# GestaltCogTeam/STEP

Measured on AMD Instinct MI355X. Metric: training windows/sec on PEMS04, horizon-12 MAE parity, 1/2/4/8 MI355X, higher is better.
Workload: dtype f16 (TSFormer Q/K/weights) + bf16 (P, V, GraphWaveNet / graph-learner GEMMs) operands, f32 accumulate

## Files before the change

include/step_hip.h:

```cpp
#ifndef STEP_HIP_H
#define STEP_HIP_H

#include <stdint.h>

#ifdef __cplusplus
extern "C" {
#endif

const char* step_last_error(void);
int step_abi_version(void);

typedef struct StepGemm {
    int M, N, K, batch;
    const void* A; long sam, sak, sab; int a_bf16;
    const void* B; long sbk, sbn, sbb; int b_bf16;
    float* C; long ldc, scn, scb;
    float alpha;
    int accumulate;
    const float* bias; int relu;
    int splitk;
    int a_kblk; long a_kstride;
    int b_kblk; long b_kstride;
    int b_nblk; long b_nstride;
    int c_nblk; long c_nstride;
// ... 37 lines not shown
    float *bn3_w, *bn3_b, *bn3_rm, *bn3_rv;
    float *fc_out_w, *fc_out_b;
    float *fc_cat_w, *fc_cat_b;
    int gemm_bf16;
} StepDglParams;

long step_dgl_global_saved_floats(int N, int T);
long step_dgl_global_work_floats(int N, int T, int backward);
int step_dgl_global_forward(const float* series_nt, int N, int T, const StepDglParams* p, int training,
                            float momentum, float* saved, float* work, float* g, void* stream);
int step_dgl_global_backward(const float* series_nt, int N, int T, const StepDglParams* p, const float* saved,
                             const float* dg, float* work, const StepDglParams* grads, void* stream);
#define STEP_DGL_FRESH_FC_GRAD 16
int step_dgl_global_backward_phase(const float* series_nt, int N, int T, const StepDglParams* p, const float* saved,
                             const float* dg, float* work, const StepDglParams* grads, int phase, void* stream);

typedef struct StepDglShard { int own1; double count1, count2; } StepDglShard;
int step_dgl_global_forward_shard(const float* series_slice, int N, int Ts, const StepDglParams* p, int training, float momentum,
                                  float* saved, float* work, double* sums, float* g, const StepDglShard* shard, int phase,
                                  void* stream);
int step_dgl_global_backward_shard(const float* series_slice, int N, int Ts, const StepDglParams* p, const float* saved,
                                   const float* dg, float* work, const StepDglParams* grads, const StepDglShard* shard, int phase,
                                   void* stream);
long step_dgl_global_offset(int N, int T, int item);

long step_dgl_edges_saved_floats(int B, int N);
long step_dgl_edges_work_floats(int N);
long step_dgl_edges_theta_offset(int N);
int step_dgl_edges_forward(const float* g, int N, int B, const StepDglParams* p, const float* u, uint64_t seed,
                           float temperature, float* saved, float* theta_out, float* adj_out, void* stream);
// ... 91 lines not shown
                               uint32_t* keepbits, const uint64_t* pool, long pool_words, void* stream);
int step_pt_attention_bwd_bf16(const uint16_t* qkv, const uint16_t* out, const uint16_t* dout, const float* stats, long S, int T, float p,
                               uint64_t seed, uint32_t site, uint16_t* dqkv, const uint32_t* keepbits, void* stream);
int step_pt_linear_bf16out(const float* x, const float* w, long swk, long swn, const float* bias, long R, int N, int K, uint16_t* out,
                           void* stream);
int step_pt_relu_mask(float* d, const float* y, long n, void* stream);
int step_colsum(const float* x, long rows, int cols, long ld, float* out, void* stream);

long step_adam_work_floats(void);
int step_adam_clip(float* params, const float* grads, float* exp_avg, float* exp_avg_sq, long n, float lr, float beta1,
                   float beta2, float eps, float weight_decay, int step, float max_norm, float* work, float* out_norm,
                   void* stream);
int step_adam_clip_sharded(float* params, const float* grads, float* exp_avg, float* exp_avg_sq, long n, float lr, float beta1,
                           float beta2, float eps, float weight_decay, int step, float max_norm, const float* extra_sumsq,
                           float* work, float* out_norm, void* stream);
int step_loss_fwd_bwd(const float* pred, const float* real, long n_pred, const float* theta, const float* prior, long n_adj,
                      float null_val, float coef, double* work, float* loss, float* dpred, float* dtheta, void* stream);
int step_loss_scaled_fwd_bwd(const float* pred, const float* real, long n_pred, long real_stride, float scale, float shift,
                             const float* theta, const float* prior, long n_adj, float null_val, float coef, double* work, float* loss,
                             float* dpred, float* dtheta, void* stream);
int step_masked_metrics(const float* pred, long pred_stride, const float* real, long real_stride, long n, float null_val, double* work,
                        float* out, void* stream);
int step_scale2(const float* a, long na, const float* b, long nb, const float* g, float* out_a, float* out_b, void* stream);

typedef struct StepDynState {
    uint64_t seed_xor;
    int32_t adam_step;
    float lr;
    float gsl_coef;
    float reserved;
// ... 67 lines not shown
```

step_amd/_lib.py:

```python
import ctypes
import os

import torch

_HERE = os.path.dirname(os.path.abspath(__file__))
LIB_PATH = os.environ.get("STEP_HIP_LIB") or os.path.join(_HERE, "libstep_hip.so")

_vp, _i, _l, _f, _u64 = ctypes.c_void_p, ctypes.c_int, ctypes.c_long, ctypes.c_float, ctypes.c_uint64


class StepGemm(ctypes.Structure):
    _fields_ = [("M", _i), ("N", _i), ("K", _i), ("batch", _i),
                ("A", _vp), ("sam", _l), ("sak", _l), ("sab", _l), ("a_bf16", _i),
                ("B", _vp), ("sbk", _l), ("sbn", _l), ("sbb", _l), ("b_bf16", _i),
                ("C", _vp), ("ldc", _l), ("scn", _l), ("scb", _l),
                ("alpha", _f), ("accumulate", _i), ("bias", _vp), ("relu", _i), ("splitk", _i),
                ("a_kblk", _i), ("a_kstride", _l), ("b_kblk", _i), ("b_kstride", _l),
                ("b_nblk", _i), ("b_nstride", _l), ("c_nblk", _i), ("c_nstride", _l),
                ("a_kscale", _vp), ("a_kshift", _vp), ("a_kperiod", _i),
                ("batch0", _i), ("sab1", _l), ("sbb1", _l), ("scb1", _l), ("compute_bf16", _i), ("a_rowsum", _vp), ("c_nscale", _vp), ("c_nshift", _vp), ("c_mvec", _vp),
                ("c_nperiod", _i), ("splitk_ws", _vp), ("splitk_ws_floats", _l)]


class StepDglParams(ctypes.Structure):
# ... 34 lines not shown
    "step_tsformer_encode": (_i, [_vp, _i, _i, _vp, _l, _i, _i, _vp, _vp, _vp, _vp, _f, _vp, _l, _u64, _vp, _vp]),
    "step_dropout_pool_fill": (_i, [_vp, _l, _f, _u64, _vp]),
    "step_tsformer_dropout_words": (_l, [_i, _i]),
    "step_gather_windows": (_i, [_vp, _i, _i, _i, _i, _vp, _i, _i, _i, _vp, _vp, _vp, _vp]),
    "step_pack_long_history": (_i, [_vp, _i, _i, _i, _i, _i, _vp, _vp]),
    "step_knn_workspace_bytes": (_l, [_i, _i, _i]),
    "step_knn_graph": (_i, [_vp, _vp, _i, _i, _i, _i, _vp, _vp, _vp, _l, _vp]),
    "step_topk_mask": (_i, [_vp, _i, _i, _i, _vp, _vp, _l, _vp]),
    "step_selftest_mfma": (_i, [_vp, _vp]),
    "step_streams_concurrent": (_i, [_vp, _vp, ctypes.POINTER(_i)]),
    "step_dgl_global_saved_floats": (_l, [_i, _i]),
    "step_dgl_global_work_floats": (_l, [_i, _i, _i]),
    "step_dgl_global_forward": (_i, [_vp, _i, _i, _PD, _i, _f, _vp, _vp, _vp, _vp]),
    "step_dgl_global_backward": (_i, [_vp, _i, _i, _PD, _vp, _vp, _vp, _PD, _vp]),
    "step_dgl_global_backward_phase": (_i, [_vp, _i, _i, _PD, _vp, _vp, _vp, _PD, _i, _vp]),
    "step_dgl_global_forward_shard": (_i, [_vp, _i, _i, _PD, _i, _f, _vp, _vp, _vp, _vp, _PS, _i, _vp]),
    "step_dgl_global_backward_shard": (_i, [_vp, _i, _i, _PD, _vp, _vp, _vp, _PD, _PS, _i, _vp]),
    "step_dgl_global_offset": (_l, [_i, _i, _i]),
    "step_dgl_edges_saved_floats": (_l, [_i, _i]),
    "step_dgl_edges_work_floats": (_l, [_i]),
    "step_dgl_edges_theta_offset": (_l, [_i]),
    "step_dgl_edges_forward": (_i, [_vp, _i, _i, _PD, _vp, _u64, _f, _vp, _vp, _vp, _vp]),
    "step_dgl_edges_forward_keyed": (_i, [_vp, _i, _i, _PD, _vp, _u64, _f, _vp, _vp, _vp, _vp]),
    "step_dgl_edges_backward": (_i, [_vp, _i, _i, _PD, _vp, _vp, _vp, _f, _vp, _PD, _vp, _vp, _vp]),
    "step_dgl_edges_backward_acc": (_i, [_vp, _i, _i, _PD, _vp, _vp, _vp, _f, _vp, _PD, _vp, _i, _vp, _vp]),
    "step_gwnet_saved_floats": (_l, [_i, _i, _i]),
    "step_gwnet_work_floats": (_l, [_i, _i, _i]),
    "step_gwnet_saved_offset": (_l, [_i, _i, _i, _i, _i]),
    "step_gwnet_forward": (_i, [_vp, _i, _i, _i, _vp, _vp, _PG, _i, _f, _u64, _f, _vp, _vp, _vp, _vp]),
    "step_gwnet_forward_phase": (_i, [_vp, _i, _i, _i, _vp, _vp, _PG, _i, _f, _u64, _f, _vp, _vp, _vp, _i, _vp]),
# ... 34 lines not shown
    "step_pt_layernorm_bwd": (_i, [_vp, _vp, _l, _vp, _vp, _vp, _vp, _vp, _vp]),
    "step_pt_attention_fwd": (_i, [_vp, _l, _i, _f, _u64, ctypes.c_uint32, _vp, _vp, _vp]),
    "step_pt_attention_bwd": (_i, [_vp, _vp, _vp, _vp, _l, _i, _f, _u64, ctypes.c_uint32, _vp, _vp]),
    "step_pt_attention_fwd_bf16": (_i, [_vp, _l, _i, _f, _u64, ctypes.c_uint32, _vp, _vp, _vp, _vp, _l, _vp]),
    "step_pt_attention_bwd_bf16": (_i, [_vp, _vp, _vp, _vp, _l, _i, _f, _u64, ctypes.c_uint32, _vp, _vp, _vp]),
    "step_pt_linear_bf16out": (_i, [_vp, _vp, _l, _l, _vp, _l, _i, _i, _vp, _vp]),
    "step_pt_relu_mask": (_i, [_vp, _vp, _l, _vp]),
    "step_colsum": (_i, [_vp, _l, _i, _l, _vp, _vp]),
    "step_loss_fwd_bwd": (_i, [_vp, _vp, _l, _vp, _vp, _l, _f, _f, _vp, _vp, _vp, _vp, _vp]),
    "step_loss_scaled_fwd_bwd": (_i, [_vp, _vp, _l, _l, _f, _f, _vp, _vp, _l, _f, _f, _vp, _vp, _vp, _vp, _vp]),
    "step_scale2": (_i, [_vp, _l, _vp, _l, _vp, _vp, _vp, _vp]),
    "step_masked_metrics": (_i, [_vp, _l, _vp, _l, _l, _f, _vp, _vp, _vp]),
    "step_adam_work_floats": (_l, []),
    "step_adam_clip": (_i, [_vp, _vp, _vp, _vp, _l, _f, _f, _f, _f, _f, _i, _f, _vp, _vp, _vp]),
    "step_adam_clip_sharded": (_i, [_vp, _vp, _vp, _vp, _l, _f, _f, _f, _f, _f, _i, _f, _vp, _vp, _vp, _vp]),
    "step_comm_available": (_i, []),
    "step_comm_version": (_i, []),
    "step_comm_unique_id": (_i, [_vp]),
    "step_comm_init_rank": (_i, [_vp, _i, _i, ctypes.POINTER(_vp)]),
    "step_comm_destroy": (_i, [_vp]),
    "step_comm_set_side_stream": (_i, [_vp, _vp]),
    "step_comm_allreduce": (_i, [_vp, _vp, _l, _i, _i, _vp]),
    "step_comm_broadcast": (_i, [_vp, _vp, _l, _i, _i, _vp]),
    "step_grad_allreduce": (_i, [_vp, _vp, _l, _vp]),
    "step_grad_allreduce_begin": (_i, [_vp, _vp, _l, _vp]),
    "step_grad_allreduce_join": (_i, [_vp, _vp]),
    "step_dyn_advance": (_i, [_vp, _vp]),
    "step_dropout_pool_fill_dyn": (_i, [_vp, _l, _f, _u64, _vp, _vp]),
    "step_dgl_edges_forward_dyn": (_i, [_vp, _i, _i, _PD, _vp, _u64, _f, _vp, _vp, _vp, _vp, _vp]),
    "step_gwnet_forward_phase_dyn": (_i, [_vp, _i, _i, _i, _vp, _vp, _PG, _i, _f, _u64, _f, _vp, _vp, _vp, _i, _vp, _vp]),
# ... 99 lines not shown
```

step_amd/csrc/dgl.hip:

```cpp
#include "common.h"
#include "step_internal.h"

namespace {

constexpr int KW = 10;
constexpr int EMB = 100;

template <int CI, int CO, int TPT>
__global__ __launch_bounds__(256) void conv_relu_fwd_kernel(const float* __restrict__ in, const float* __restrict__ w,
                                                            const float* __restrict__ b, const float* __restrict__ in_sc,
                                                            const float* __restrict__ in_sh, float* __restrict__ out,
                                                            float* __restrict__ partial, int Tin, int stat_limit) {
    __shared__ __attribute__((aligned(16))) float ws[CI * KW * CO];
    __shared__ float red[4][2 * CO];
    const int tid = threadIdx.x, n = blockIdx.y;
    const int Tout = Tin - (KW - 1);
    for (int e = tid; e < CI * KW * CO; e += 256) {
        int co = e % CO, k = (e / CO) % KW, ci = e / (CO * KW);
        ws[e] = w[(co * CI + ci) * KW + k];
    }
    __syncthreads();
    const int t0 = (blockIdx.x * 256 + tid) * TPT;
    float acc[CO][TPT];
#pragma unroll
// ... 156 lines not shown
            rvar[j] = (1.f - momentum) * rvar[j] + momentum * (float)(var * N / fmax((double)N - 1.0, 1.0));
        }
    } else {
        mean = rmean[j]; var = rvar[j];
    }
    const float rstd = (float)(1.0 / sqrt(var + 1e-5));
    if (tid == 0) { stat[2 * EMB + j] = (float)mean; stat[3 * EMB + j] = rstd; }
    const float sc = gamma[j] * rstd, sh = beta[j] - (float)mean * sc;
    for (int n = tid; n < N; n += 256) g[(long)n * EMB + j] = fmaxf(gpre[(long)n * EMB + j], 0.f) * sc + sh;
}

__global__ __launch_bounds__(256) void bn3_relu_bwd_kernel(const float* __restrict__ dg, const float* __restrict__ gpre, int N,
                                                           const float* __restrict__ gamma, const float* __restrict__ stat,
                                                           float* __restrict__ dgamma, float* __restrict__ dbeta,
                                                           float* __restrict__ dbias, float* __restrict__ dgpre,
                                                           float* __restrict__ dgpreT, float* __restrict__ colsum) {
    __shared__ double r1[256], r2[256];
    const int j = blockIdx.x, tid = threadIdx.x;
    const float mean = stat[2 * EMB + j], rstd = stat[3 * EMB + j];
    double a = 0.0, q = 0.0;
    for (int n = tid; n < N; n += 256) {
        float d = dg[(long)n * EMB + j];
        float xh = (fmaxf(gpre[(long)n * EMB + j], 0.f) - mean) * rstd;
        a += d; q += (double)d * xh;
    }
    r1[tid] = a; r2[tid] = q;
    __syncthreads();
    for (int s = 128; s > 0; s >>= 1) {
        if (tid < s) { r1[tid] += r1[tid + s]; r2[tid] += r2[tid + s]; }
        __syncthreads();
    }
    const float m1 = (float)(r1[0] / N), m2 = (float)(r2[0] / N);
    const float k = gamma[j] * rstd;
// ... 422 lines not shown
        uint4* dst = wp + ((long)o * T2 + t) * 2;
        dst[0] = make_uint4(pack_bf16x2(v[0], v[1]), pack_bf16x2(v[2], v[3]), pack_bf16x2(v[4], v[5]), pack_bf16x2(v[6], v[7]));
        dst[1] = make_uint4(pack_bf16x2(v[8], v[9]), pack_bf16x2(v[10], v[11]), pack_bf16x2(v[12], v[13]), pack_bf16x2(v[14], v[15]));
    }
    acc = wave_sum(acc);
    if ((tid & 63) == 0) red[tid >> 6] = acc;
    __syncthreads();
    if (tid == 0) atomicAdd(&shiftdot[o], red[0] + red[1] + red[2] + red[3]);
}
__global__ void gpre_init_kernel(float* __restrict__ gpre, const float* __restrict__ shiftdot, long n) {
    const long i = (long)blockIdx.x * 256 + threadIdx.x;
    if (i < n) gpre[i] = shiftdot[i % EMB];
}
__global__ __launch_bounds__(256) void fc_unpermute_kernel(const float* __restrict__ graw, const float* __restrict__ fc_w,
                                                           const float* __restrict__ st2, const float* __restrict__ colsum,
                                                           float* __restrict__ dfc_w, float* __restrict__ dots_o, int T2, int overwrite) {
    __shared__ float red[16][32];
    const int o = blockIdx.y, t = blockIdx.x * 256 + threadIdx.x, tid = threadIdx.x, lane = tid & 63, wave = tid >> 6;
    const float cso = colsum[o];
    float d[32];
#pragma unroll
    for (int i = 0; i < 32; ++i) d[i] = 0.f;
    if (t < T2) {
        const float4* src = (const float4*)(graw + ((long)o * T2 + t) * 16);
        const float4 g0 = src[0], g1 = src[1], g2 = src[2], g3 = src[3];
        const float g[16] = {g0.x, g0.y, g0.z, g0.w, g1.x, g1.y, g1.z, g1.w, g2.x, g2.y, g2.z, g2.w, g3.x, g3.y, g3.z, g3.w};
        float w[16], old[16];
#pragma unroll
        for (int c = 0; c < 16; ++c) { const long idx = ((long)o * 16 + c) * T2 + t; w[c] = fc_w[idx]; old[c] = overwrite ? 0.f : dfc_w[idx]; }
#pragma unroll
        for (int c = 0; c < 16; ++c) {
            dfc_w[((long)o * 16 + c) * T2 + t] = old[c] + st2[c] * g[c] + st2[16 + c] * cso;
            d[2 * c] = w[c] * g[c]; d[2 * c + 1] = w[c] * cso;
        }
    }
#pragma unroll
    for (int i = 0; i < 32; ++i) {
        const float v = row_sum_fast(d[i]);
        if ((lane & 15) == 15) red[4 * wave + (lane >> 4)][i] = v;
    }
    __syncthreads();
    if (tid < 32) {
        float v = 0.f;
#pragma unroll
        for (int r = 0; r < 16; ++r) v += red[r][tid];
        atomicAdd(&dots_o[o * 32 + tid], v);
    }
}
__global__ void dots_reduce_kernel(const float* __restrict__ dots_o, float* __restrict__ dots) {
    const int i = threadIdx.x;
    if (i >= 32) return;
    double a = 0.0;
    for (int o = 0; o < EMB; ++o) a += dots_o[o * 32 + i];
    dots[i] = (float)a;
}

static bool dgl_channels_last(const StepDglParams* p) {
    const char* e = getenv("STEP_DGL_F32_STORAGE");
    return p->gemm_bf16 && !(e && e[0] == '1');
}

static bool dgl_legacy_bn_backward() {
// ... 143 lines not shown
}

extern "C" long step_dgl_global_offset(int N, int T, int item) {
    const long T1 = T - 9, T2 = T - 18;
    if (item == 0) return 0;
    if (item == 1) return (long)N * 8 * T1;
    if (item == 2) return (long)N * 8 * T1 + (long)N * 16 * T2;
    const long nb1 = (long)N * cdiv(T1, 1024), nb2 = (long)N * cdiv(T2, 1024);
    const long coef = (nb1 > nb2 ? nb1 : nb2) * 32 + 64 + (long)N * 16 * T2 + (long)N * 8 * T1 + wraw_floats(T2) + 2L * N * EMB;
    if (item == 10) return coef + 256;
    if (item == 11) return coef + 320;
    return -1;
}

static int dgl_global_backward_impl(const float* series_nt, int N, int T, const StepDglParams* p, const float* saved, const float* dg,
                                    float* work, const StepDglParams* grads, const StepDglShard* shard, int phase, void* stream);

extern "C" int step_dgl_global_backward(const float* series_nt, int N, int T, const StepDglParams* p, const float* saved,
                                        const float* dg, float* work, const StepDglParams* grads, void* stream) {
    return step_dgl_global_backward_phase(series_nt, N, T, p, saved, dg, work, grads, 0, stream);
}

extern "C" int step_dgl_global_backward_phase(const float* series_nt, int N, int T, const StepDglParams* p, const float* saved,
                                              const float* dg, float* work, const StepDglParams* grads, int phase, void* stream) {
    STEP_REQUIRE(series_nt && p && saved && dg && work && grads && N > 0 && T > 18 && (phase & ~STEP_DGL_FRESH_FC_GRAD) >= 0 &&
                 (phase & ~STEP_DGL_FRESH_FC_GRAD) <= 2, "dgl_global_backward: bad arguments");
    return dgl_global_backward_impl(series_nt, N, T, p, saved, dg, work, grads, nullptr, phase, stream);
}

extern "C" int step_dgl_global_backward_shard(const float* series_slice, int N, int Ts, const StepDglParams* p, const float* saved,
                                              const float* dg, float* work, const StepDglParams* grads, const StepDglShard* shard,
                                              int phase, void* stream) {
    const int ph = phase & ~STEP_DGL_FRESH_FC_GRAD;
    STEP_REQUIRE(series_slice && p && saved && dg && work && grads && shard && N > 0 && Ts > 18 && (ph == 1 || ph == 3 || ph == 4),
                 "dgl_global_backward_shard: bad arguments");
    STEP_REQUIRE(p->gemm_bf16 && Ts - 18 >= 128, "dgl_global_backward_shard: needs the bf16 contraction mode and a slice of >= 128 conv2 columns");
    return dgl_global_backward_impl(series_slice, N, Ts, p, saved, dg, work, grads, shard, phase, stream);
}

static int dgl_global_backward_impl(const float* series_nt, int N, int T, const StepDglParams* p, const float* saved, const float* dg,
                                    float* work, const StepDglParams* grads, const StepDglShard* shard, int phase, void* stream) {
    const int fresh_fc = (phase & STEP_DGL_FRESH_FC_GRAD) ? 1 : 0;
    phase &= ~STEP_DGL_FRESH_FC_GRAD;
    const bool do_fc = phase == 0 || phase == 1, do_mid = phase == 0 || phase == 2 || phase == 3, do_tail = phase == 0 || phase == 2 || phase == 4;
    hipStream_t st = (hipStream_t)stream;
    const int T1 = T - 9, T2 = T - 18;
    const long K = 16L * T2;
    float *a1, *a2, *gpre, *st1, *st2, *st3;
    carve_saved((float*)saved, N, T, &a1, &a2, &gpre, &st1, &st2, &st3);
    long nb1 = (long)N * cdiv(T1, 1024), nb2 = (long)N * cdiv(T2, 1024);
    float* partial = work;
    float* d_a2 = work + (nb1 > nb2 ? nb1 : nb2) * 32 + 64;
    float* d_a1 = d_a2 + (long)N * 16 * T2;
    float* wraw = d_a1 + (long)N * 8 * T1;
    float* dgpre = wraw + wraw_floats(T2);
    float* dgpreT = dgpre + (long)N * EMB;
    float* coef = dgpreT + (long)N * EMB;
    float* dots = coef + 256;
    float* graw = coef + 320;
    float* wg_scratch = coef + DGL_SMALL;
    const bool fuse2 = T2 >= 128 && (shard || !dgl_legacy_bn_backward());
    const double count1 = shard ? shard->count1 : (double)N * T1, count2 = shard ? shard->count2 : (double)N * T2;
    if (dgl_channels_last(p)) {
        const float* wp = saved_wp((float*)saved, N, T);
        float* dots_o = coef + 256 + 64 + 1344;
        float* colsum = coef + 128;
        if (do_fc) {
            bn3_relu_bwd_kernel<<<EMB, 256, 0, st>>>(dg, gpre, N, p->bn3_w, st3, grads->bn3_w, grads->bn3_b, grads->fc_b, dgpre, dgpreT, colsum);
            STEP_LAUNCH_CHECK("bn3_bwd");
            StepGemm gm = gemm_desc(EMB, (int)K, N, dgpre, 1, EMB, a2, K, 1, wraw, K);
            gm.b_bf16 = 1;
            gm.compute_bf16 = 1;
            STEP_TRY(step_gemm_launch(gm, st));
            if (hipMemsetAsync(dots_o, 0, EMB * 32 * sizeof(float), st) != hipSuccess) { step_set_error("memset failed"); return STEP_ERR_HIP; }
            fc_unpermute_kernel<<<dim3(cdiv(T2, 256), EMB), 256, 0, st>>>(wraw, p->fc_w, st2, colsum, grads->fc_w, dots_o, T2, fresh_fc);
            dots_reduce_kernel<<<1, 64, 0, st>>>(dots_o, dots);
            STEP_LAUNCH_CHECK("fc_unpermute");
        }
        if (do_mid) {
            bn2_fused_coef_kernel<<<1, 64, 0, st>>>(dots, st2, p->bn2_w, count2, grads->bn2_w, grads->bn2_b, coef);
            STEP_LAUNCH_CHECK("bn2_fused_coef");
            StepGemm gm = gemm_desc(N, (int)K, EMB, dgpre, EMB, 1, wp, K, 1, d_a2, K);
            gm.b_bf16 = 1;
            gm.compute_bf16 = 1;
            GemmFused fu = {nullptr, nullptr, a2, coef, st2, 16, T2, GEMM_FUSED_INTERLEAVED};
            STEP_TRY(step_gemm_launch_fused(gm, fu, st));
            STEP_TRY(dgl_conv2_wgrad_cl(d_a2, a1, wg_scratch, graw, N, T1, st));
        }
        if (do_tail) {
            STEP_TRY(dgl_conv2_wgrad_finish(graw, p->conv2_w, st1, p->bn1_w, p->bn1_b, count1, grads->conv2_w, grads->conv2_b, grads->bn1_w,
                                            grads->bn1_b, coef + 64, 1, st));
            STEP_TRY(dgl_conv2_dgrad_cl(d_a2, p->conv2_w, st1, d_a1, N, T1, a1, coef + 64, st1, shard ? shard->own1 : T1, wraw, st));
            STEP_TRY(dgl_conv1_wgrad_cl(d_a1, series_nt, wg_scratch, grads->conv1_w, grads->conv1_b, N, T, st));
        }
        return STEP_OK;
    }
    if (do_fc) {
        float* colsum = coef + 128;
        bn3_relu_bwd_kernel<<<EMB, 256, 0, st>>>(dg, gpre, N, p->bn3_w, st3, grads->bn3_w, grads->bn3_b, grads->fc_b, dgpre, dgpreT, colsum);
        STEP_LAUNCH_CHECK("bn3_bwd");
        {
            StepGemm gm = gemm_desc(EMB, (int)K, N, dgpre, 1, EMB, a2, K, 1, grads->fc_w, K);
            gm.accumulate = fresh_fc ? 0 : 1;
            gm.c_nscale = st2; gm.c_nshift = st2 + 16; gm.c_nperiod = T2; gm.c_mvec = colsum;
            gm.compute_bf16 = p->gemm_bf16;
            if (fuse2) {
                if (hipMemsetAsync(dots, 0, 32 * sizeof(float), st) != hipSuccess) { step_set_error("memset failed"); return STEP_ERR_HIP; }
                GemmFused fu = {p->fc_w, dots, nullptr, nullptr, nullptr, 16, T2};
                STEP_TRY(step_gemm_launch_fused(gm, fu, st));
            } else {
                STEP_TRY(step_gemm_launch(gm, st));
            }
        }
    }
// ... 175 lines not shown
```

step_amd/csrc/optim.hip:

```cpp
#include "common.h"
#include "step_internal.h"
#include "tail_device.h"

namespace {

constexpr int NB = 1024;

__global__ __launch_bounds__(256) void sumsq_partial_kernel(const float* __restrict__ g, long n, float* __restrict__ partial) {
    __shared__ float red[4];
    float s = 0.f;
    const long n4 = n / 4;
    const float4* g4 = (const float4*)g;
    for (long i = (long)blockIdx.x * 256 + threadIdx.x; i < n4; i += (long)gridDim.x * 256) {
        float4 v = g4[i];
        s += v.x * v.x + v.y * v.y + v.z * v.z + v.w * v.w;
    }
    if (blockIdx.x == 0)
        for (long i = n4 * 4 + threadIdx.x; i < n; i += 256) s += g[i] * g[i];
    s = wave_sum(s);
    if ((threadIdx.x & 63) == 0) red[threadIdx.x >> 6] = s;
    __syncthreads();
    if (threadIdx.x == 0) partial[blockIdx.x] = red[0] + red[1] + red[2] + red[3];
}

__global__ __launch_bounds__(256) void adam_clip_kernel(float* __restrict__ p, const float* __restrict__ g, float* __restrict__ m,
                                                        float* __restrict__ v, long n, float lr, float beta1, float beta2, float eps,
                                                        float wd, float bc1, float bc2_sqrt, float max_norm,
                                                        const float* __restrict__ partial, int npartial, const float* __restrict__ extra_sumsq,
                                                        float* __restrict__ out_norm, const StepDynState* __restrict__ dyn) {
    __shared__ float red[4];
    __shared__ float s_coef;
    if (dyn) {
        const float t = (float)dyn->adam_step;
        lr = dyn->lr;
        bc1 = 1.f - powf(beta1, t);
        bc2_sqrt = sqrtf(1.f - powf(beta2, t));
    }
    {
        float s = 0.f;
        for (int i = threadIdx.x; i < npartial; i += 256) s += partial[i];
        s = wave_sum(s);
        if ((threadIdx.x & 63) == 0) red[threadIdx.x >> 6] = s;
        __syncthreads();
        if (threadIdx.x == 0) {
            const bool given = max_norm < 0.f;
            const float mx = given ? -max_norm : max_norm;
            const float norm = sqrtf(given ? *extra_sumsq : red[0] + red[1] + red[2] + red[3] + (extra_sumsq ? *extra_sumsq : 0.f));
            float c = mx > 0.f ? mx / (norm + 1e-6f) : 1.f;
            s_coef = c < 1.f ? c : 1.f;
            if (out_norm && blockIdx.x == 0) *out_norm = norm;
        }
        __syncthreads();
    }
    const float coef = s_coef;
    const float step_size = lr / bc1;
    for (long i = (long)blockIdx.x * 256 + threadIdx.x; i < n; i += (long)gridDim.x * 256) {
        const float pi = p[i];
        const float gi = g[i] * coef + wd * pi;
        const float mi = beta1 * m[i] + (1.f - beta1) * gi;
        const float vi = beta2 * v[i] + (1.f - beta2) * gi * gi;
        m[i] = mi; v[i] = vi;
        p[i] = pi - step_size * mi / (sqrtf(vi) / bc2_sqrt + eps);
// ... 1 lines not shown
}

}

extern "C" long step_adam_work_floats(void) { return NB + 8; }

extern "C" int step_adam_clip(float* params, const float* grads, float* exp_avg, float* exp_avg_sq, long n, float lr, float beta1,
                              float beta2, float eps, float weight_decay, int step, float max_norm, float* work, float* out_norm,
                              void* stream) {
    return step_adam_clip_sharded(params, grads, exp_avg, exp_avg_sq, n, lr, beta1, beta2, eps, weight_decay, step, max_norm, nullptr, work,
                                  out_norm, stream);
}

static int adam_clip_launch(float* params, const float* grads, float* exp_avg, float* exp_avg_sq, long n, float lr, float beta1,
                            float beta2, float eps, float weight_decay, int step, float max_norm, const float* extra_sumsq,
                            float* work, float* out_norm, const StepDynState* dyn, void* stream);
extern "C" int step_adam_clip_sharded(float* params, const float* grads, float* exp_avg, float* exp_avg_sq, long n, float lr, float beta1,
                                      float beta2, float eps, float weight_decay, int step, float max_norm, const float* extra_sumsq,
                                      float* work, float* out_norm, void* stream) {
    return adam_clip_launch(params, grads, exp_avg, exp_avg_sq, n, lr, beta1, beta2, eps, weight_decay, step, max_norm, extra_sumsq, work, out_norm,
                            nullptr, stream);
}
extern "C" int step_adam_clip_dyn(float* params, const float* grads, float* exp_avg, float* exp_avg_sq, long n, float beta1, float beta2,
                                  float eps, float weight_decay, float max_norm, const float* extra_sumsq, float* work, float* out_norm,
                                  const StepDynState* dyn, void* stream) {
    STEP_REQUIRE(dyn, "adam_clip_dyn: null state");
    return adam_clip_launch(params, grads, exp_avg, exp_avg_sq, n, 0.f, beta1, beta2, eps, weight_decay, 1, max_norm, extra_sumsq, work, out_norm, dyn,
                            stream);
}
__global__ void dyn_advance_kernel(StepDynState* s) {
    uint64_t z = s->seed_xor + 0x9E3779B97F4A7C15ull;
    z = (z ^ (z >> 30)) * 0xBF58476D1CE4E5B9ull;
    z = (z ^ (z >> 27)) * 0x94D049BB133111EBull;
    s->seed_xor = z ^ (z >> 31);
    s->adam_step += 1;
}
extern "C" int step_dyn_advance(StepDynState* dyn, void* stream) {
    STEP_REQUIRE(dyn, "dyn_advance: null state");
    dyn_advance_kernel<<<1, 1, 0, (hipStream_t)stream>>>(dyn);
    STEP_LAUNCH_CHECK("dyn_advance");
    return STEP_OK;
}
static int adam_clip_launch(float* params, const float* grads, float* exp_avg, float* exp_avg_sq, long n, float lr, float beta1,
                            float beta2, float eps, float weight_decay, int step, float max_norm, const float* extra_sumsq,
                            float* work, float* out_norm, const StepDynState* dyn, void* stream) {
    STEP_REQUIRE(params && grads && exp_avg && exp_avg_sq && work && n > 0 && step >= 1, "adam_clip: bad arguments");
    STEP_REQUIRE((((uintptr_t)grads) & 15) == 0, "adam_clip: gradient buffer must be 16-byte aligned");
    STEP_REQUIRE(max_norm >= 0.f || extra_sumsq, "adam_clip: max_norm < 0 (squared norm supplied by the caller) needs extra_sumsq");
    hipStream_t st = (hipStream_t)stream;
    sumsq_partial_kernel<<<NB, 256, 0, st>>>(grads, n, work);
    STEP_LAUNCH_CHECK("sumsq_partial");
    const float bc1 = 1.f - powf(beta1, (float)step);
    const float bc2 = 1.f - powf(beta2, (float)step);
    int blocks = (int)((n + 255) / 256);
    if (blocks > 4096) blocks = 4096;
    adam_clip_kernel<<<blocks, 256, 0, st>>>(params, grads, exp_avg, exp_avg_sq, n, lr, beta1, beta2, eps, weight_decay, bc1, sqrtf(bc2),
                                             max_norm, work, NB, extra_sumsq, out_norm, dyn);
    STEP_LAUNCH_CHECK("adam_clip");
    return STEP_OK;
}

namespace {
__global__ __launch_bounds__(256) void loss_reduce_kernel(const float* __restrict__ pred, const float* __restrict__ real, long n1, long rs,
                                                          float scale, float shift,
                                                          const float* __restrict__ theta, const float* __restrict__ prior, long n2,
                                                          float null_val, double* __restrict__ acc ) {
    __shared__ double red[4][3];
    double s_abs = 0.0, s_cnt = 0.0, s_bce = 0.0;
    const long stride = (long)gridDim.x * 256;
    for (long i = (long)blockIdx.x * 256 + threadIdx.x; i < n1; i += stride) {
        const TailElem e = tail_rescale(pred[i], real[i * rs], scale, shift, null_val);
        if (e.m) {
// ... 140 lines not shown
```

step_amd/optim.py:

```python
import torch

from . import _lib
from .step_arch.discrete_graph_learning import cut_time_columns, paste_time_columns


def flat_items(model):
    if hasattr(model, "_pt_params"):
        items, off = [], 0
        for n, p in zip(model._pt_names, model._pt_params()):
            items.append((n, off, p))
            off += (p.numel() + 3) & ~3
        return items
    lay, tr = model._grad_layout(), dict(model._trainable())
    return [(k, lay["items"][k][0], tr[k]) for k in lay["order"]]


def index_flat_items(items, params, names=None):
    params = list(params)
    pos = {}
    for i, p in enumerate(params):
        pos.setdefault(id(p), i)
    missing = [n for n, _, p in items if id(p) not in pos]
    if missing:
        raise ValueError(f"FusedAdamClip: params lacks {len(missing)} parameter(s) of the flat buffer (first: {missing[0]!r}): pass every "
# ... 176 lines not shown
        if hasattr(self.model, "_drop_eval_g"):
            self.model._drop_eval_g()
        extra = None
        max_norm = float(self.max_norm or 0.0)
        sh = getattr(getattr(self.model, "discrete_graph_learning", None), "_shard", None)
        if sh is not None:
            extra = self.model._other_slices_sumsq
            if max_norm > 0.0 and self.dyn is None and getattr(self.model, "_total_sumsq", None) is not None:
                extra, max_norm = self.model._total_sumsq, -max_norm
        if self.dyn is not None:
            _lib.call("step_adam_clip_dyn", _lib.ptr(self.flat), _lib.ptr(g), _lib.ptr(self.exp_avg), _lib.ptr(self.exp_avg_sq),
                      self.flat.numel(), float(pg["betas"][0]), float(pg["betas"][1]), float(pg["eps"]), float(pg["weight_decay"]),
                      float(self.max_norm or 0.0), _lib.ptr(extra), _lib.ptr(self.work), _lib.ptr(self.grad_norm), _lib.ptr(self.dyn),
                      _lib.stream())
            return
        _lib.call("step_adam_clip_sharded", _lib.ptr(self.flat), _lib.ptr(g), _lib.ptr(self.exp_avg), _lib.ptr(self.exp_avg_sq),
                  self.flat.numel(), float(pg["lr"]), float(pg["betas"][0]), float(pg["betas"][1]), float(pg["eps"]),
                  float(pg["weight_decay"]), self.step_count, max_norm, _lib.ptr(extra), _lib.ptr(self.work),
                  _lib.ptr(self.grad_norm), _lib.stream())

    def state_dict(self):
        if self._index is None:
            groups = [{k: v for k, v in g.items() if k != "params"} for g in self.param_groups]
            return {"step": self.step_count, "exp_avg": self.exp_avg, "exp_avg_sq": self.exp_avg_sq, "param_groups": groups}
        gathered = None
        if self._sliced is not None and self.step_count > 0:
            gathered = self._staging
            if gathered is None:
                raise RuntimeError("FusedAdamClip: the graph learner is sharded in time slices and this optimizer has stepped since the "
                                   "last gather: call gather_state() on ALL ranks (e.g. in the runner's on_epoch_end) before "
# ... 46 lines not shown
```

step_amd/step_arch/step.py:

```python
import ctypes
import os

import torch
from torch import nn

from .. import _lib
from .tsformer import TSFormer
from .graphwavenet import GraphWaveNet, fill_gwnet_struct
from .discrete_graph_learning import DiscreteGraphLearning, fill_dgl_struct
from . import eval_cache as _ec

TEMPERATURE = 0.5
BN_MOMENTUM = 0.1


def _f32(n, device):
    return torch.empty(int(n), device=device, dtype=torch.float32)


class LongHistoryRef:

    def __init__(self, data, t0, length, channels=None, t0_host=None):
        assert data.is_cuda and data.dtype == torch.float32 and data.dim() == 3 and data.is_contiguous()
        assert t0.is_cuda and t0.dtype == torch.int64 and t0.dim() == 1
# ... 237 lines not shown
        use_aux = model.overlap_streams and os.environ.get("STEP_NO_AUX", "0") != "1"
        aux = ctypes.c_void_p(model._side_stream(dev, "aux").cuda_stream) if use_aux else None
        leaf = ctypes.c_void_p(model._side_stream(dev, "leaf").cuda_stream) if (use_aux and os.environ.get("STEP_LEAF_STREAM", "0") == "1") else None
        joined = [False]

        def join_aux():
            if aux is not None:
                torch.cuda.current_stream().wait_stream(model._side_stream(dev, "aux"))
            if leaf is not None:
                torch.cuda.current_stream().wait_stream(model._side_stream(dev, "leaf"))
            joined[0] = True
        if esaved._version != ctx.esaved_version:
            raise RuntimeError("step_amd.STEP: the returned edge probabilities (theta) were modified in place after forward(); the native "
                               "backward reads that buffer -- use an out-of-place op (theta.clamp(...)) or theta.clone()")
        FRESH = 16
        try:
            L.call("step_gwnet_backward", L.ptr(hist), B, N, Cin, L.ptr(last), ctypes.byref(bstruct), L.ptr(wsaved), L.ptr(wwork),
                   L.ptr(dpred), ctypes.byref(gw_grads), L.ptr(dadj), int(drop > 0), aux, leaf, st)
            ework = _f32(L.lib().step_dgl_edges_work_floats(N), dev)
            dth = dtheta.contiguous().float() if dtheta is not None else None
            if grp is None:
                dgv = _f32(N * 100, dev)
                L.call("step_dgl_edges_backward", L.ptr(g), N, B, ctypes.byref(dstruct), L.ptr(esaved), L.ptr(dth) if dth is not None else None,
                       L.ptr(dadj), TEMPERATURE, L.ptr(ework), ctypes.byref(dg_grads), L.ptr(dgv), leaf if leaf is not None else aux, st)
            else:
                if nth == 1:
                    grp["dg"] = _f32(N * 100, dev)
                dgv = grp["dg"]
                L.call("step_dgl_edges_backward_acc", L.ptr(g), N, B, ctypes.byref(dstruct), L.ptr(esaved), L.ptr(dth) if dth is not None else None,
                       L.ptr(dadj), TEMPERATURE, L.ptr(ework), ctypes.byref(dg_grads), L.ptr(dgv), int(nth > 1), leaf if leaf is not None else aux, st)
            gwork = _f32(L.lib().step_dgl_global_work_floats(N, Ttr, 1), dev) if final else None
            fo, fn, _ = layout["items"]["dgl.fc_w"]
            assert fo + fn == layout["total"] or fo + ((fn + 3) & ~3) == layout["total"]
            assert layout["norm_slot"] == fo - 4
            sh = dgl._shard
            if not final:
                join_aux()
            elif sh is None:
                L.call("step_dgl_global_backward_phase", L.ptr(dgl._series_nt), N, Ttr, ctypes.byref(dstruct), L.ptr(gsaved), L.ptr(dgv),
                       L.ptr(gwork), ctypes.byref(dg_grads), 1 | FRESH, st)
                pending = model._reduce_begin(flat[fo:fo + fn])
                L.call("step_dgl_global_backward_phase", L.ptr(dgl._series_nt), N, Ttr, ctypes.byref(dstruct), L.ptr(gsaved), L.ptr(dgv),
                       L.ptr(gwork), ctypes.byref(dg_grads), 2, st)
                join_aux()
                pending += model._reduce_begin(flat[:fo])
                model._reduce_finish(flat, pending, flat)
            else:
                world = sh["world"]
                model._sum_over_ranks(dgv)
                dgv.mul_(1.0 / world)
                dgl._slice_dirty = True
                sstruct = dgl.shard_struct()
                o_dots, o_graw = L.lib().step_dgl_global_offset(N, Ttr, 10), L.lib().step_dgl_global_offset(N, Ttr, 11)
                exchange = {1: gwork[o_dots:o_dots + 32], 3: gwork[o_graw:o_graw + 1296]}
                for phase in (1, 3, 4):
                    L.call("step_dgl_global_backward_shard", L.ptr(dgl._series_slice), N, Ttr, ctypes.byref(dstruct), L.ptr(gsaved), L.ptr(dgv),
                           L.ptr(gwork), ctypes.byref(dg_grads), ctypes.byref(sstruct), phase | FRESH, st)
                    if phase in exchange:
                        model._sum_over_ranks(exchange[phase])
# ... 3 lines not shown
                ns = layout["norm_slot"]
                own = torch.linalg.vector_norm(flat[fo:fo + fn]).reshape(1)
                torch.mul(own.square(), float(world), out=flat[ns:ns + 1])
                model._reduce_finish(flat, model._reduce_begin(flat[:fo]), flat[:fo])
                model._other_slices_sumsq = torch.addcmul(flat[ns:ns + 1], own, own, value=-1.0)
                slices = flat[ns:ns + 1].clone()
                flat[ns:ns + 1].zero_()
                rep = torch.linalg.vector_norm(flat[:fo])
                model._total_sumsq = torch.addcmul(slices, rep, rep)
        finally:
            if not joined[0]:
                join_aux()
        del wwork, ework
        model._flat_grad = flat
        model._backward_count = getattr(model, "_backward_count", 0) + 1
        model._drop_eval_g()
        ctx.held = None
        del views, gw_grads, dg_grads
        if model.flat_gradients_only or nth > 1:
            return (None, None, None, None) + (None,) * len(layout["order"])
        return (None, None, None, None) + tuple(flat[o:o + n].view(shape) for o, n, shape in (layout["items"][k] for k in layout["order"]))


_STREAMS = {}


def _concurrent_stream(dev, tries=8, priority=0):
    if os.environ.get("STEP_STREAM_PROBE", "1") == "0":
        return torch.cuda.Stream(device=dev, priority=priority)
    main = torch.cuda.current_stream(dev)
# ... 42 lines not shown
        self._noise_key = None
        self._dyn = None
        self._process_group = None
        self._struct_cache = {}
        self._bwd_cache = None
        self._trainable_cache = None
        self.flat_gradients_only = False
        self._comm = None
        self._min_world = 1
        self._layout = None
        self._zg_params = None
        self._zg_key = None
        self._last = {}
        self._flat_param = None
        self._flat_grad = None
        self._backward_count = 0
        self.overlap_streams = os.environ.get("STEP_NO_OVERLAP", "0") != "1"
        self.split_wavenet_prep = os.environ.get("STEP_PREP_SPLIT", "0") == "1"
        self.prefetch_knn_stream = os.environ.get("STEP_PREFETCH_KNN_STREAM", "0") == "1"
        self._prefetched = None
        self._precision_override = None
        self.prefetch_fifo = 2
        self._alias = {}
        self.prefetch_enabled = os.environ.get("STEP_NO_PREFETCH", "0") != "1"
        self._reduce_wait_ms = None
        self._reduce_events = []
        self._small_events = []
        self.eval_cache_bytes = 0
        self._eval_cache_chunk_windows = 256
        self.eval_cache_stats = _ec.new_stats()
# ... 420 lines not shown
        from .. import comm as _comm
        self._comm = _comm.open_transport(self._process_group, collectives, self.backend.nodevec1.device, self._min_world)
        if self._comm is not None:
            self._comm.use_side_stream(self._side_stream(self.backend.nodevec1.device, "comm"))
        if sync_module_states and dist.get_world_size(self._process_group) > self._min_world:
            _comm.broadcast_module_states(self, self._process_group)
        if shard_graph_learner and dist.get_world_size(self._process_group) > self._min_world:
            if self.matmul_precision != "bf16":
                raise ValueError("shard_graph_learner needs matmul_precision = 'bf16' (the sliced backward uses the fused BatchNorm backward)")
            self.discrete_graph_learning.shard_time_slices(dist.get_rank(self._process_group), dist.get_world_size(self._process_group))
            self._layout = None
            self._flat_param = None
            self._zg_params = None
            self._struct_cache, self._bwd_cache, self._trainable_cache = {}, None, None

    def _reduce_begin(self, chunk):
        if self._process_group is None:
            return []
        import torch.distributed as dist
        if dist.get_world_size(self._process_group) <= self._min_world or chunk.numel() == 0:
            return []
        if self._comm is not None:
            self._comm.grad_allreduce_begin(chunk)
            return [None]
        return [dist.all_reduce(chunk, group=self._process_group, async_op=True)]

    def _sum_over_ranks(self, t):
        import torch.distributed as dist
        if self._process_group is not None and dist.get_world_size(self._process_group) > self._min_world:
            timed = self._reduce_wait_ms is not None and t.is_cuda
# ... 46 lines not shown
    def _reduce_flat_grads(self, flat):
        self._reduce_finish(flat, self._reduce_begin(flat), flat)

    def zero_grad(self, set_to_none=True):
        if set_to_none:
            key = self._module_key()
            ps = self._zg_params
            if ps is None or self._zg_key != key:
                ps = self._zg_params = list(self.parameters())
                self._zg_key = key
            for q in ps:
                q.grad = None
        else:
            super().zero_grad(set_to_none=False)
        self._flat_grad = None
        self._backward_count = 0
        self._group_open = False
        self._acc = None

    def train(self, mode=True):
        if bool(mode) != self.training and self._prefetched:
            self.cancel_prefetch()
        if mode:
            self._eval_g = None
        return super().train(mode)

    def _apply(self, fn, recurse=True):
        self._zg_params = None
        self._struct_cache, self._bwd_cache, self._trainable_cache = {}, None, None
        self._invalidate_eval_cache()
# ... 47 lines not shown
```

Baseline: 2407.

## Fuse fc_w gradient sum-of-squares into unpermute kernel for partial clip norm

The fc_unpermute kernel now accumulates the squared norm of the freshly written fc_w gradient into a double scalar. Adam's clip norm then only reduces the gradients outside the fc block and adds this precomputed value, so the large fc_w gradient is not re-read for the norm. The memset of dots_o is folded into the bn3 backward kernel, which also zeroes the sumsq scalar. This path is limited to the single-process bf16 channels-last mode and adds version checks so the offer is only used when the flat gradient is unchanged. Per-block double atomics and partial-norm bookkeeping are added in exchange.

```diff
diff --git a/include/step_hip.h b/include/step_hip.h
--- a/include/step_hip.h
+++ b/include/step_hip.h
@@ -75,6 +75,8 @@
 #define STEP_DGL_FRESH_FC_GRAD 16
 int step_dgl_global_backward_phase(const float* series_nt, int N, int T, const StepDglParams* p, const float* saved,
                              const float* dg, float* work, const StepDglParams* grads, int phase, void* stream);
+int step_dgl_global_backward_sumsq(const float* series_nt, int N, int T, const StepDglParams* p, const float* saved,
+                                   const float* dg, float* work, const StepDglParams* grads, int phase, double* fc_sumsq, void* stream);
 
 typedef struct StepDglShard { int own1; double count1, count2; } StepDglShard;
 int step_dgl_global_forward_shard(const float* series_slice, int N, int Ts, const StepDglParams* p, int training, float momentum,
@@ -196,6 +198,9 @@
 int step_adam_clip_sharded(float* params, const float* grads, float* exp_avg, float* exp_avg_sq, long n, float lr, float beta1,
                            float beta2, float eps, float weight_decay, int step, float max_norm, const float* extra_sumsq,
                            float* work, float* out_norm, void* stream);
+int step_adam_clip_partial_norm(float* params, const float* grads, float* exp_avg, float* exp_avg_sq, long n, long n_norm, float lr,
+                                float beta1, float beta2, float eps, float weight_decay, int step, float max_norm,
+                                const double* extra_sumsq, float* work, float* out_norm, void* stream);
 int step_loss_fwd_bwd(const float* pred, const float* real, long n_pred, const float* theta, const float* prior, long n_adj,
                       float null_val, float coef, double* work, float* loss, float* dpred, float* dtheta, void* stream);
 int step_loss_scaled_fwd_bwd(const float* pred, const float* real, long n_pred, long real_stride, float scale, float shift,
diff --git a/step_amd/_lib.py b/step_amd/_lib.py
--- a/step_amd/_lib.py
+++ b/step_amd/_lib.py
@@ -72,6 +72,7 @@
     "step_dgl_global_forward": (_i, [_vp, _i, _i, _PD, _i, _f, _vp, _vp, _vp, _vp]),
     "step_dgl_global_backward": (_i, [_vp, _i, _i, _PD, _vp, _vp, _vp, _PD, _vp]),
     "step_dgl_global_backward_phase": (_i, [_vp, _i, _i, _PD, _vp, _vp, _vp, _PD, _i, _vp]),
+    "step_dgl_global_backward_sumsq": (_i, [_vp, _i, _i, _PD, _vp, _vp, _vp, _PD, _i, _vp, _vp]),
     "step_dgl_global_forward_shard": (_i, [_vp, _i, _i, _PD, _i, _f, _vp, _vp, _vp, _vp, _PS, _i, _vp]),
     "step_dgl_global_backward_shard": (_i, [_vp, _i, _i, _PD, _vp, _vp, _vp, _PD, _PS, _i, _vp]),
     "step_dgl_global_offset": (_l, [_i, _i, _i]),
@@ -136,6 +137,7 @@
     "step_adam_work_floats": (_l, []),
     "step_adam_clip": (_i, [_vp, _vp, _vp, _vp, _l, _f, _f, _f, _f, _f, _i, _f, _vp, _vp, _vp]),
     "step_adam_clip_sharded": (_i, [_vp, _vp, _vp, _vp, _l, _f, _f, _f, _f, _f, _i, _f, _vp, _vp, _vp, _vp]),
+    "step_adam_clip_partial_norm": (_i, [_vp, _vp, _vp, _vp, _l, _l, _f, _f, _f, _f, _f, _i, _f, _vp, _vp, _vp, _vp]),
     "step_comm_available": (_i, []),
     "step_comm_version": (_i, []),
     "step_comm_unique_id": (_i, [_vp]),
diff --git a/step_amd/csrc/dgl.hip b/step_amd/csrc/dgl.hip
--- a/step_amd/csrc/dgl.hip
+++ b/step_amd/csrc/dgl.hip
@@ -194,9 +194,12 @@
                                                            const float* __restrict__ gamma, const float* __restrict__ stat,
                                                            float* __restrict__ dgamma, float* __restrict__ dbeta,
                                                            float* __restrict__ dbias, float* __restrict__ dgpre,
-                                                           float* __restrict__ dgpreT, float* __restrict__ colsum) {
+                                                           float* __restrict__ dgpreT, float* __restrict__ colsum,
+                                                           float* __restrict__ zero_rows, double* __restrict__ zero1) {
     __shared__ double r1[256], r2[256];
     const int j = blockIdx.x, tid = threadIdx.x;
+    if (zero_rows && tid < 32) zero_rows[j * 32 + tid] = 0.f;
+    if (j == 0 && zero1 && tid == 32) *zero1 = 0.0;
     const float mean = stat[2 * EMB + j], rstd = stat[3 * EMB + j];
     double a = 0.0, q = 0.0;
     for (int n = tid; n < N; n += 256) {
@@ -649,11 +652,13 @@
 }
 __global__ __launch_bounds__(256) void fc_unpermute_kernel(const float* __restrict__ graw, const float* __restrict__ fc_w,
                                                            const float* __restrict__ st2, const float* __restrict__ colsum,
-                                                           float* __restrict__ dfc_w, float* __restrict__ dots_o, int T2, int overwrite) {
+                                                           float* __restrict__ dfc_w, float* __restrict__ dots_o, double* __restrict__ sumsq,
+                                                           int T2, int overwrite) {
     __shared__ float red[16][32];
     const int o = blockIdx.y, t = blockIdx.x * 256 + threadIdx.x, tid = threadIdx.x, lane = tid & 63, wave = tid >> 6;
     const float cso = colsum[o];
     float d[32];
+    float sq = 0.f;
 #pragma unroll
     for (int i = 0; i < 32; ++i) d[i] = 0.f;
     if (t < T2) {
@@ -665,9 +670,16 @@
         for (int c = 0; c < 16; ++c) { const long idx = ((long)o * 16 + c) * T2 + t; w[c] = fc_w[idx]; old[c] = overwrite ? 0.f : dfc_w[idx]; }
 #pragma unroll
         for (int c = 0; c < 16; ++c) {
-            dfc_w[((long)o * 16 + c) * T2 + t] = old[c] + st2[c] * g[c] + st2[16 + c] * cso;
+            const float v = old[c] + st2[c] * g[c] + st2[16 + c] * cso;
+            dfc_w[((long)o * 16 + c) * T2 + t] = v;
+            sq += v * v;
             d[2 * c] = w[c] * g[c]; d[2 * c + 1] = w[c] * cso;
         }
+    }
+    __shared__ float sqw[4];
+    if (sumsq) {
+        sq = wave_sum_fast(sq);
+        if (lane == 0) sqw[wave] = sq;
     }
 #pragma unroll
     for (int i = 0; i < 32; ++i) {
@@ -681,6 +693,7 @@
         for (int r = 0; r < 16; ++r) v += red[r][tid];
         atomicAdd(&dots_o[o * 32 + tid], v);
     }
+    if (sumsq && tid == 32) atomicAdd(sumsq, (double)sqw[0] + (double)sqw[1] + (double)sqw[2] + (double)sqw[3]);
 }
 __global__ void dots_reduce_kernel(const float* __restrict__ dots_o, float* __restrict__ dots) {
     const int i = threadIdx.x;
@@ -854,7 +867,8 @@
 }
 
 static int dgl_global_backward_impl(const float* series_nt, int N, int T, const StepDglParams* p, const float* saved, const float* dg,
-                                    float* work, const StepDglParams* grads, const StepDglShard* shard, int phase, void* stream);
+                                    float* work, const StepDglParams* grads, const StepDglShard* shard, int phase, double* fc_sumsq,
+                                    void* stream);
 
 extern "C" int step_dgl_global_backward(const float* series_nt, int N, int T, const StepDglParams* p, const float* saved,
                                         const float* dg, float* work, const StepDglParams* grads, void* stream) {
@@ -865,7 +879,16 @@
                                               const float* dg, float* work, const StepDglParams* grads, int phase, void* stream) {
     STEP_REQUIRE(series_nt && p && saved && dg && work && grads && N > 0 && T > 18 && (phase & ~STEP_DGL_FRESH_FC_GRAD) >= 0 &&
                  (phase & ~STEP_DGL_FRESH_FC_GRAD) <= 2, "dgl_global_backward: bad arguments");
-    return dgl_global_backward_impl(series_nt, N, T, p, saved, dg, work, grads, nullptr, phase, stream);
+    return dgl_global_backward_impl(series_nt, N, T, p, saved, dg, work, grads, nullptr, phase, nullptr, stream);
+}
+
+extern "C" int step_dgl_global_backward_sumsq(const float* series_nt, int N, int T, const StepDglParams* p, const float* saved,
+                                              const float* dg, float* work, const StepDglParams* grads, int phase, double* fc_sumsq,
+                                              void* stream) {
+    STEP_REQUIRE(series_nt && p && saved && dg && work && grads && fc_sumsq && N > 0 && T > 18 && (phase & ~STEP_DGL_FRESH_FC_GRAD) >= 0 &&
+                 (phase & ~STEP_DGL_FRESH_FC_GRAD) <= 2, "dgl_global_backward_sumsq: bad arguments");
+    STEP_REQUIRE(dgl_channels_last(p), "dgl_global_backward_sumsq: needs the bf16 mode's channels-last storage");
+    return dgl_global_backward_impl(series_nt, N, T, p, saved, dg, work, grads, nullptr, phase, fc_sumsq, stream);
 }
 
 extern "C" int step_dgl_global_backward_shard(const float* series_slice, int N, int Ts, const StepDglParams* p, const float* saved,
@@ -875,11 +898,12 @@
     STEP_REQUIRE(series_slice && p && saved && dg && work && grads && shard && N > 0 && Ts > 18 && (ph == 1 || ph == 3 || ph == 4),
                  "dgl_global_backward_shard: bad arguments");
     STEP_REQUIRE(p->gemm_bf16 && Ts - 18 >= 128, "dgl_global_backward_shard: needs the bf16 contraction mode and a slice of >= 128 conv2 columns");
-    return dgl_global_backward_impl(series_slice, N, Ts, p, saved, dg, work, grads, shard, phase, stream);
+    return dgl_global_backward_impl(series_slice, N, Ts, p, saved, dg, work, grads, shard, phase, nullptr, stream);
 }
 
 static int dgl_global_backward_impl(const float* series_nt, int N, int T, const StepDglParams* p, const float* saved, const float* dg,
-                                    float* work, const StepDglParams* grads, const StepDglShard* shard, int phase, void* stream) {
+                                    float* work, const StepDglParams* grads, const StepDglShard* shard, int phase, double* fc_sumsq,
+                                    void* stream) {
     const int fresh_fc = (phase & STEP_DGL_FRESH_FC_GRAD) ? 1 : 0;
     phase &= ~STEP_DGL_FRESH_FC_GRAD;
     const bool do_fc = phase == 0 || phase == 1, do_mid = phase == 0 || phase == 2 || phase == 3, do_tail = phase == 0 || phase == 2 || phase == 4;
@@ -906,14 +930,14 @@
         float* dots_o = coef + 256 + 64 + 1344;
         float* colsum = coef + 128;
         if (do_fc) {
-            bn3_relu_bwd_kernel<<<EMB, 256, 0, st>>>(dg, gpre, N, p->bn3_w, st3, grads->bn3_w, grads->bn3_b, grads->fc_b, dgpre, dgpreT, colsum);
+            bn3_relu_bwd_kernel<<<EMB, 256, 0, st>>>(dg, gpre, N, p->bn3_w, st3, grads->bn3_w, grads->bn3_b, grads->fc_b, dgpre, dgpreT, colsum,
+                                                     dots_o, fc_sumsq);
             STEP_LAUNCH_CHECK("bn3_bwd");
             StepGemm gm = gemm_desc(EMB, (int)K, N, dgpre, 1, EMB, a2, K, 1, wraw, K);
             gm.b_bf16 = 1;
             gm.compute_bf16 = 1;
             STEP_TRY(step_gemm_launch(gm, st));
-            if (hipMemsetAsync(dots_o, 0, EMB * 32 * sizeof(float), st) != hipSuccess) { step_set_error("memset failed"); return STEP_ERR_HIP; }
-            fc_unpermute_kernel<<<dim3(cdiv(T2, 256), EMB), 256, 0, st>>>(wraw, p->fc_w, st2, colsum, grads->fc_w, dots_o, T2, fresh_fc);
+            fc_unpermute_kernel<<<dim3(cdiv(T2, 256), EMB), 256, 0, st>>>(wraw, p->fc_w, st2, colsum, grads->fc_w, dots_o, fc_sumsq, T2, fresh_fc);
             dots_reduce_kernel<<<1, 64, 0, st>>>(dots_o, dots);
             STEP_LAUNCH_CHECK("fc_unpermute");
         }
@@ -937,7 +961,8 @@
     }
     if (do_fc) {
         float* colsum = coef + 128;
-        bn3_relu_bwd_kernel<<<EMB, 256, 0, st>>>(dg, gpre, N, p->bn3_w, st3, grads->bn3_w, grads->bn3_b, grads->fc_b, dgpre, dgpreT, colsum);
+        bn3_relu_bwd_kernel<<<EMB, 256, 0, st>>>(dg, gpre, N, p->bn3_w, st3, grads->bn3_w, grads->bn3_b, grads->fc_b, dgpre, dgpreT, colsum, nullptr,
+                                                 nullptr);
         STEP_LAUNCH_CHECK("bn3_bwd");
         {
             StepGemm gm = gemm_desc(EMB, (int)K, N, dgpre, 1, EMB, a2, K, 1, grads->fc_w, K);
diff --git a/step_amd/csrc/optim.hip b/step_amd/csrc/optim.hip
--- a/step_amd/csrc/optim.hip
+++ b/step_amd/csrc/optim.hip
@@ -27,7 +27,8 @@
                                                         float* __restrict__ v, long n, float lr, float beta1, float beta2, float eps,
                                                         float wd, float bc1, float bc2_sqrt, float max_norm,
                                                         const float* __restrict__ partial, int npartial, const float* __restrict__ extra_sumsq,
-                                                        float* __restrict__ out_norm, const StepDynState* __restrict__ dyn) {
+                                                        const double* __restrict__ extra64, float* __restrict__ out_norm,
+                                                        const StepDynState* __restrict__ dyn) {
     __shared__ float red[4];
     __shared__ float s_coef;
     if (dyn) {
@@ -45,7 +46,8 @@
         if (threadIdx.x == 0) {
             const bool given = max_norm < 0.f;
             const float mx = given ? -max_norm : max_norm;
-            const float norm = sqrtf(given ? *extra_sumsq : red[0] + red[1] + red[2] + red[3] + (extra_sumsq ? *extra_sumsq : 0.f));
+            const float own = red[0] + red[1] + red[2] + red[3];
+            const float norm = sqrtf(given ? *extra_sumsq : extra64 ? (float)((double)own + *extra64) : own + (extra_sumsq ? *extra_sumsq : 0.f));
             float c = mx > 0.f ? mx / (norm + 1e-6f) : 1.f;
             s_coef = c < 1.f ? c : 1.f;
             if (out_norm && blockIdx.x == 0) *out_norm = norm;
@@ -77,19 +79,26 @@
 
 static int adam_clip_launch(float* params, const float* grads, float* exp_avg, float* exp_avg_sq, long n, float lr, float beta1,
                             float beta2, float eps, float weight_decay, int step, float max_norm, const float* extra_sumsq,
-                            float* work, float* out_norm, const StepDynState* dyn, void* stream);
+                            float* work, float* out_norm, const StepDynState* dyn, long n_norm, const double* extra64, void* stream);
 extern "C" int step_adam_clip_sharded(float* params, const float* grads, float* exp_avg, float* exp_avg_sq, long n, float lr, float beta1,
                                       float beta2, float eps, float weight_decay, int step, float max_norm, const float* extra_sumsq,
                                       float* work, float* out_norm, void* stream) {
     return adam_clip_launch(params, grads, exp_avg, exp_avg_sq, n, lr, beta1, beta2, eps, weight_decay, step, max_norm, extra_sumsq, work, out_norm,
-                            nullptr, stream);
+                            nullptr, n, nullptr, stream);
+}
+extern "C" int step_adam_clip_partial_norm(float* params, const float* grads, float* exp_avg, float* exp_avg_sq, long n, long n_norm, float lr,
+                                           float beta1, float beta2, float eps, float weight_decay, int step, float max_norm,
+                                           const double* extra_sumsq, float* work, float* out_norm, void* stream) {
+    STEP_REQUIRE(extra_sumsq && n_norm > 0 && n_norm <= n && max_norm >= 0.f, "adam_clip_partial_norm: bad arguments");
+    return adam_clip_launch(params, grads, exp_avg, exp_avg_sq, n, lr, beta1, beta2, eps, weight_decay, step, max_norm, nullptr, work, out_norm,
+                            nullptr, n_norm, extra_sumsq, stream);
 }
 extern "C" int step_adam_clip_dyn(float* params, const float* grads, float* exp_avg, float* exp_avg_sq, long n, float beta1, float beta2,
                                   float eps, float weight_decay, float max_norm, const float* extra_sumsq, float* work, float* out_norm,
                                   const StepDynState* dyn, void* stream) {
     STEP_REQUIRE(dyn, "adam_clip_dyn: null state");
     return adam_clip_launch(params, grads, exp_avg, exp_avg_sq, n, 0.f, beta1, beta2, eps, weight_decay, 1, max_norm, extra_sumsq, work, out_norm, dyn,
-                            stream);
+                            n, nullptr, stream);
 }
 __global__ void dyn_advance_kernel(StepDynState* s) {
     uint64_t z = s->seed_xor + 0x9E3779B97F4A7C15ull;
@@ -106,19 +115,19 @@
 }
 static int adam_clip_launch(float* params, const float* grads, float* exp_avg, float* exp_avg_sq, long n, float lr, float beta1,
                             float beta2, float eps, float weight_decay, int step, float max_norm, const float* extra_sumsq,
-                            float* work, float* out_norm, const StepDynState* dyn, void* stream) {
+                            float* work, float* out_norm, const StepDynState* dyn, long n_norm, const double* extra64, void* stream) {
     STEP_REQUIRE(params && grads && exp_avg && exp_avg_sq && work && n > 0 && step >= 1, "adam_clip: bad arguments");
     STEP_REQUIRE((((uintptr_t)grads) & 15) == 0, "adam_clip: gradient buffer must be 16-byte aligned");
     STEP_REQUIRE(max_norm >= 0.f || extra_sumsq, "adam_clip: max_norm < 0 (squared norm supplied by the caller) needs extra_sumsq");
     hipStream_t st = (hipStream_t)stream;
-    sumsq_partial_kernel<<<NB, 256, 0, st>>>(grads, n, work);
+    sumsq_partial_kernel<<<NB, 256, 0, st>>>(grads, n_norm, work);
     STEP_LAUNCH_CHECK("sumsq_partial");
     const float bc1 = 1.f - powf(beta1, (float)step);
     const float bc2 = 1.f - powf(beta2, (float)step);
     int blocks = (int)((n + 255) / 256);
     if (blocks > 4096) blocks = 4096;
     adam_clip_kernel<<<blocks, 256, 0, st>>>(params, grads, exp_avg, exp_avg_sq, n, lr, beta1, beta2, eps, weight_decay, bc1, sqrtf(bc2),
-                                             max_norm, work, NB, extra_sumsq, out_norm, dyn);
+                                             max_norm, work, NB, extra_sumsq, extra64, out_norm, dyn);
     STEP_LAUNCH_CHECK("adam_clip");
     return STEP_OK;
 }
diff --git a/step_amd/optim.py b/step_amd/optim.py
--- a/step_amd/optim.py
+++ b/step_amd/optim.py
@@ -214,6 +214,13 @@
                       float(self.max_norm or 0.0), _lib.ptr(extra), _lib.ptr(self.work), _lib.ptr(self.grad_norm), _lib.ptr(self.dyn),
                       _lib.stream())
             return
+        offer = getattr(self.model, "_fc_sumsq", None)
+        if offer is not None and sh is None and offer[2] is g and g._version == offer[3] and 0 < offer[1] < g.numel():
+            _lib.call("step_adam_clip_partial_norm", _lib.ptr(self.flat), _lib.ptr(g), _lib.ptr(self.exp_avg), _lib.ptr(self.exp_avg_sq),
+                      self.flat.numel(), int(offer[1]), float(pg["lr"]), float(pg["betas"][0]), float(pg["betas"][1]), float(pg["eps"]),
+                      float(pg["weight_decay"]), self.step_count, max_norm, _lib.ptr(offer[0]), _lib.ptr(self.work),
+                      _lib.ptr(self.grad_norm), _lib.stream())
+            return
         _lib.call("step_adam_clip_sharded", _lib.ptr(self.flat), _lib.ptr(g), _lib.ptr(self.exp_avg), _lib.ptr(self.exp_avg_sq),
                   self.flat.numel(), float(pg["lr"]), float(pg["betas"][0]), float(pg["betas"][1]), float(pg["eps"]),
                   float(pg["weight_decay"]), self.step_count, max_norm, _lib.ptr(extra), _lib.ptr(self.work),
diff --git a/step_amd/step_arch/step.py b/step_amd/step_arch/step.py
--- a/step_amd/step_arch/step.py
+++ b/step_amd/step_arch/step.py
@@ -275,6 +275,7 @@
             raise RuntimeError("step_amd.STEP: the returned edge probabilities (theta) were modified in place after forward(); the native "
                                "backward reads that buffer -- use an out-of-place op (theta.clamp(...)) or theta.clone()")
         FRESH = 16
+        fc_sumsq_offer = None
         try:
             L.call("step_gwnet_backward", L.ptr(hist), B, N, Cin, L.ptr(last), ctypes.byref(bstruct), L.ptr(wsaved), L.ptr(wwork),
                    L.ptr(dpred), ctypes.byref(gw_grads), L.ptr(dadj), int(drop > 0), aux, leaf, st)
@@ -298,12 +299,20 @@
             if not final:
                 join_aux()
             elif sh is None:
-                L.call("step_dgl_global_backward_phase", L.ptr(dgl._series_nt), N, Ttr, ctypes.byref(dstruct), L.ptr(gsaved), L.ptr(dgv),
-                       L.ptr(gwork), ctypes.byref(dg_grads), 1 | FRESH, st)
+                cl = bf == 1 and os.environ.get("STEP_DGL_F32_STORAGE", "0")[:1] != "1"
+                sumsq = model._fc_sumsq_scalar(dev) if (model._process_group is None and cl) else None
+                if sumsq is not None:
+                    L.call("step_dgl_global_backward_sumsq", L.ptr(dgl._series_nt), N, Ttr, ctypes.byref(dstruct), L.ptr(gsaved), L.ptr(dgv),
+                           L.ptr(gwork), ctypes.byref(dg_grads), 1 | FRESH, L.ptr(sumsq), st)
+                else:
+                    L.call("step_dgl_global_backward_phase", L.ptr(dgl._series_nt), N, Ttr, ctypes.byref(dstruct), L.ptr(gsaved), L.ptr(dgv),
+                           L.ptr(gwork), ctypes.byref(dg_grads), 1 | FRESH, st)
                 pending = model._reduce_begin(flat[fo:fo + fn])
                 L.call("step_dgl_global_backward_phase", L.ptr(dgl._series_nt), N, Ttr, ctypes.byref(dstruct), L.ptr(gsaved), L.ptr(dgv),
                        L.ptr(gwork), ctypes.byref(dg_grads), 2, st)
                 join_aux()
+                if sumsq is not None:
+                    fc_sumsq_offer = (sumsq, fo)
                 pending += model._reduce_begin(flat[:fo])
                 model._reduce_finish(flat, pending, flat)
             else:
@@ -337,6 +346,7 @@
         del wwork, ework
         model._flat_grad = flat
         model._backward_count = getattr(model, "_backward_count", 0) + 1
+        model._fc_sumsq = None if fc_sumsq_offer is None else fc_sumsq_offer + (flat, flat._version)
         model._drop_eval_g()
         ctx.held = None
         del views, gw_grads, dg_grads
@@ -409,6 +419,7 @@
         self._last = {}
         self._flat_param = None
         self._flat_grad = None
+        self._fc_sumsq = None
         self._backward_count = 0
         self.overlap_streams = os.environ.get("STEP_NO_OVERLAP", "0") != "1"
         self.split_wavenet_prep = os.environ.get("STEP_PREP_SPLIT", "0") == "1"
@@ -859,6 +870,12 @@
             self._zg_params = None
             self._struct_cache, self._bwd_cache, self._trainable_cache = {}, None, None
 
+    def _fc_sumsq_scalar(self, dev):
+        t = getattr(self, "_fc_sumsq_buf", None)
+        if t is None or t.device != dev:
+            t = self._fc_sumsq_buf = torch.zeros(1, dtype=torch.float64, device=dev)
+        return t
+
     def _reduce_begin(self, chunk):
         if self._process_group is None:
             return []
@@ -935,6 +952,7 @@
         else:
             super().zero_grad(set_to_none=False)
         self._flat_grad = None
+        self._fc_sumsq = None
         self._backward_count = 0
         self._group_open = False
         self._acc = None
```

After: 2419 (median of 6 runs). No clear change (+0.5%).
